# sneppy/pokerl

Measured on AMD Instinct MI355X. Metric: env-steps/sec (whole node) + showdown hand-evals/sec, 65 536 tables 6-max, higher is better.
Workload: dtype f64; 1 GPU; 65536 tables/GPU x 1 GPU(s), num_players=6, random agents in-kernel (Philox4x32-10), start_credits=100 blinds 1/2, auto-reset; BASELINE configs[2]; tables_per_gpu=65536, num_players=6, policy=random, kernel=k_rollout_tab<6> fused, 723 steps/launch, parallelism=env-parallel, 1 shard(s), no collective on the step path

## Files before the change

pokerl_amd/csrc/pk_device.hpp:

```cpp
#pragma once
#ifndef PK_HOST_SIM
#include <hip/hip_runtime.h>
#endif
#include <stdint.h>

#include <type_traits>
#include <utility>

#include "../../include/pokerl_hip.h"

namespace pk {

enum : int { HR_SF = 1, HR_POKER = 2, HR_FULL = 3, HR_FLUSH = 4, HR_STRAIGHT = 5, HR_TRIS = 6, HR_TWO_PAIR = 7, HR_PAIR = 8, HR_HIGH = 9, HR_NONE = 10 };
enum : int { MV_FOLD = 0, MV_CHECK = 1, MV_CALL = 2, MV_RAISE_ANY = 3, MV_ALL_IN = 6 };
enum : int { PS_FOLDED = 0, PS_ACTIVE = 1, PS_CALLED = 2, PS_ALL_IN = 3, PS_BROKEN = 4 };
constexpr uint32_t STREAM_DECK = 0x4445434Bu, STREAM_ACTION = 0x41435432u;
constexpr uint32_t NONE_V = (uint32_t)HR_NONE << 20;

constexpr int EVAL7_TAB_WORDS = 8192;

struct State {
    double *credits, *bets, *pending, *payoffs;
    double *min_raise;
    uint64_t *seat_states;
// ... 484 lines not shown
__device__ __forceinline__ uint32_t eval_tab_bits(uint64_t bits, const uint32_t *T, int &nk) {
    const Eval7Front f = eval7_tab_front_bits(bits, T);
    return eval_tab_back<SEVEN, true>(f, T, nk);
}
template <bool SEVEN = false>
__device__ __forceinline__ bool tab_bits_of(uint64_t w, int n, uint64_t &bits) {
    uint32_t lo = (uint32_t)w, hi = (uint32_t)(w >> 32) & 0x00ffffffu;
    if (!SEVEN) {
        const uint32_t r4 = rep4(lo), ulo = n >= 4 ? 0xffffffffu : ((1u << ((8 * n) & 31)) - 1u);
        const uint32_t uhi = n <= 4 ? 0u : ((1u << ((8 * (n - 4)) & 31)) - 1u);
        lo = (lo & ulo) | (r4 & ~ulo); hi = ((hi & uhi) | (r4 & ~uhi)) & 0x00ffffffu;
    }
    bits = (4ull << (lo & 63)) | (4ull << ((lo >> 8) & 63)) | (4ull << ((lo >> 16) & 63)) | (4ull << ((lo >> 24) & 63)) |
           (4ull << (hi & 63)) | (4ull << ((hi >> 8) & 63)) | (4ull << ((hi >> 16) & 63));
    const bool cards_ok = ((lo & 0xc0c0c0c0u) | (hi & 0x00c0c0c0u)) == 0 && (((uint32_t)bits | (uint32_t)(bits >> 32)) & 0x80038003u) == 0;
    return (SEVEN || n >= 3) && cards_ok && __popcll(bits) == (SEVEN ? 7 : n);
}
__device__ __forceinline__ uint32_t eval_small(uint64_t w, int n, int &nk) {
    uint32_t r0 = (uint32_t)w & 0xf, r1 = (uint32_t)(w >> 8) & 0xf;
    r0 = r0 ? r0 : 13u; r1 = r1 ? r1 : 13u;
    const uint32_t hi = r0 > r1 ? r0 : r1, lo = r0 > r1 ? r1 : r0;
    const bool pair = n == 2 && r0 == r1;
    nk = n == 0 ? 0 : ((n == 1 || pair) ? 1 : 2);
    const uint32_t v2 = pair ? (((uint32_t)HR_PAIR << 20) | r0) : (((uint32_t)HR_HIGH << 20) | (hi << 4) | lo);
    return n == 0 ? NONE_V : (n == 1 ? (((uint32_t)HR_HIGH << 20) | r0) : v2);
}
__device__ __forceinline__ uint32_t eval_tab_n(const uint32_t (&c)[7], int n, const uint32_t *T, int &nk) {
    uint64_t bits = 0;
#pragma unroll
    for (int i = 0; i < 7; ++i) bits |= (i < n) ? (4ull << (c[i] & 63)) : 0ull;
    return eval_tab_bits(bits, T, nk);
}
__device__ __forceinline__ bool distinct_valid_cards(const uint32_t (&c)[7], int n) {
    uint64_t bits = 0;
    bool ok = n >= 3;
#pragma unroll
    for (int i = 0; i < 7; ++i) {
        const bool used = i < n;
        ok = ok && (!used || (c[i] < 0x40u && (c[i] & 15u) < 13u));
        bits |= used ? (1ull << (c[i] & 63)) : 0ull;
    }
    return ok && __popcll(bits) == n;
}

#ifndef PK_WAVE
#define PK_WAVE 64
#endif
#define PK_STOCK (PK_WAVE >= 4 ? 4 : 1)
#if PK_WAVE >= 16
__device__ __forceinline__ uint32_t lane_read(uint32_t v, int lane) { return (uint32_t)__builtin_amdgcn_readlane((int)v, lane); }
__device__ __forceinline__ uint64_t lane_read64(uint64_t v, int lane) { return (uint64_t)lane_read((uint32_t)v, lane) | ((uint64_t)lane_read((uint32_t)(v >> 32), lane) << 32); }
__device__ __forceinline__ bool wave_uniform(bool b) { return __builtin_amdgcn_readfirstlane((int)b) != 0; }
#endif

enum : int { PF_ACTION = 0, PF_CURSOR = 1, PF_END_PRE = 2, PF_EVAL = 3, PF_SIDEPOT = 4, PF_SETUP = 5, PF_DEAL = 6, PF_OTHER = 7,
             PF_N_CURSOR = 8, PF_N_END = 9, PF_N_EVALPASS = 10, PF_N_SIDEPOT = 11,
             PF_N_SIDEPOT_LANES = 12, PF_N_END_LANES = 13, PF_SLOTS = 16 };
#ifdef PK_PROFILE
struct Prof {
    unsigned long long acc[PF_SLOTS] = {0}, t0 = 0;
    __device__ __forceinline__ void start() { t0 = __builtin_readcyclecounter(); }
    __device__ __forceinline__ void lap(int slot) { unsigned long long t = __builtin_readcyclecounter(); acc[slot] += t - t0; t0 = t; }
    __device__ __forceinline__ void count(int slot, unsigned n = 1) { acc[slot] += n; }
    __device__ __forceinline__ void count_wave(unsigned long long *dst, int slot_events, int slot_lanes) {
        const unsigned long long act = __ballot(1);
        if ((int)(threadIdx.x & 63) == __ffsll((long long)act) - 1) {
            atomicAdd(&dst[slot_events], 1ull); atomicAdd(&dst[slot_lanes], (unsigned long long)__popcll(act));
        }
    }
    __device__ __forceinline__ void flush(unsigned long long *dst) {
        if ((threadIdx.x & 63) == 0) for (int i = 0; i < PF_SLOTS; ++i) atomicAdd(&dst[i], acc[i]);
    }
};
#define PK_PROF(x) x
#else
#define PK_PROF(x)
#endif

template <int N>
struct Lds {
    static constexpr bool TAB = false;
    uint32_t item[64 * N + 64][2];
    uint32_t res[64 * N];
    uint32_t act[8][64];
    uint32_t show[N][64];
    Fresh fresh;
    alignas(16) uint8_t nth[128][8];
    uint32_t lone[(5 + 2 * N + 3) / 4];
    uint32_t stock[PK_STOCK][(5 + 2 * N + 3) / 4];
};

template <int N, bool RING>
struct LdsTab;
template <int N>
struct LdsTab<N, true> {
    static constexpr bool TAB = true, PAIRS = false;
    uint32_t item[64 * N + 1][2];
    uint32_t act[8][64];
    uint32_t show[N][64];
    Fresh fresh;
    alignas(16) uint8_t nth[128][8];
    alignas(16) uint32_t evtab[EVAL7_TAB_WORDS];
};
template <int N>
struct LdsTab<N, false> {
    static constexpr bool TAB = true, PAIRS = true;
// ... 26 lines not shown
    bool primed = false;
    template <typename LDS>
    __device__ __forceinline__ uint32_t draw16(LDS &lds, const Hot &S, uint32_t table_id, uint64_t step_serial, bool need) {
        const int lane = threadIdx.x & (PK_WAVE - 1);
        const uint64_t qfull = step_serial >> 3;
        const uint32_t q = (uint32_t)qfull;
        if (!primed || (int32_t)(filled - q) < 0) filled = q;
        primed = true;
        if (__any(need && filled == q)) {
#pragma unroll 1
            for (int r = 0; r < 2; ++r) {
                const bool fill = (int32_t)(filled - q) < 2;
                if (!__any(fill)) break;
                if (fill) {
                    const uint64_t b = qfull + (uint64_t)(filled - q);
                    uint32_t w[4];
                    philox4x32_10(table_id, (uint32_t)b, STREAM_ACTION, (uint32_t)(b >> 32), S.key0, S.key1, w);
                    const int slot = (filled & 1) * 4;
                    lds.act[slot + 0][lane] = w[0]; lds.act[slot + 1][lane] = w[1];
                    lds.act[slot + 2][lane] = w[2]; lds.act[slot + 3][lane] = w[3];
                    filled += 1;
                }
            }
        }
        const uint32_t j = (uint32_t)step_serial & 7;
        return lds.act[(q & 1) * 4 + (j >> 1)][lane];
    }
    template <typename LDS>
    __device__ __forceinline__ void ensure(LDS &lds, const Hot &S, uint32_t table_id, uint64_t step_serial, bool may, int ahead) {
        const int lane = threadIdx.x & (PK_WAVE - 1);
        const uint64_t qfull = step_serial >> 3;
        const uint32_t q = (uint32_t)qfull;
        if (!primed || (int32_t)(filled - q) < 0) filled = q;
        primed = true;
        const int have = (int)(filled - q) * 8 - (int)((uint32_t)step_serial & 7);
        if (__any(may && have < ahead)) {
#pragma unroll 1
            for (int r = 0; r < 2; ++r) {
                const bool fill = (int32_t)(filled - q) < 2;
                if (!__any(fill)) break;
                if (fill) {
                    const uint64_t b = qfull + (uint64_t)(filled - q);
                    uint32_t w[4];
                    philox4x32_10(table_id, (uint32_t)b, STREAM_ACTION, (uint32_t)(b >> 32), S.key0, S.key1, w);
                    const int slot = (filled & 1) * 4;
                    lds.act[slot + 0][lane] = w[0]; lds.act[slot + 1][lane] = w[1];
                    lds.act[slot + 2][lane] = w[2]; lds.act[slot + 3][lane] = w[3];
                    filled += 1;
                }
            }
        }
    }
    template <typename LDS>
    __device__ __forceinline__ static uint32_t peek(const LDS &lds, uint64_t step_serial) {
        const uint32_t s = (uint32_t)step_serial;
        return lds.act[((s >> 3) & 1) * 4 + ((s & 7) >> 1)][threadIdx.x & (PK_WAVE - 1)];
    }
    __device__ __forceinline__ static uint32_t half_of(uint32_t word, uint64_t step_serial) {
        return ((uint32_t)step_serial & 1) ? (word >> 16) : (word & 0xffffu);
    }
};
struct alignas(16) NthTable {
    uint8_t e[128][8];
    constexpr NthTable() : e{} {
        for (int m = 0; m < 128; ++m) {
            int rest = m;
            for (int k = 0; k < 8; ++k) {
                int low = 0;
                while (rest && !((rest >> low) & 1)) ++low;
                e[m][k] = rest ? (uint8_t)low : (uint8_t)0;
                rest &= rest - 1;
            }
        }
    }
};
__device__ __constant__ const NthTable g_nth{};
template <typename LDS>
__device__ __forceinline__ void stage_nth(LDS &lds) {
    static_assert(alignof(NthTable) >= 16 && sizeof(NthTable) == 64 * sizeof(uint4), "stage_nth copies the table as 64 uint4");
    for (int i = threadIdx.x & (PK_WAVE - 1); i < 64; i += PK_WAVE)
        reinterpret_cast<uint4 *>(&lds.nth[0][0])[i] = reinterpret_cast<const uint4 *>(&g_nth.e[0][0])[i];
    __syncthreads();
}
template <typename LDS>
__device__ __forceinline__ int action_from_draw_lds(const LDS &lds, uint32_t r16, uint32_t mask) {
    return lds.nth[mask & 127][__umul24(r16, (uint32_t)__popc(mask)) >> 16];
}
__device__ __forceinline__ int action_from_draw(uint32_t r16, uint32_t mask) {
    uint32_t k = __umul24(r16, (uint32_t)__popc(mask)) >> 16;
    uint32_t m = mask;
#pragma unroll
    for (uint32_t i = 0; i < 6; ++i) m = (i < k) ? (m & (m - 1)) : m;
    return __ffs(m) - 1;
}

__device__ __forceinline__ int call_action(uint32_t mask) {
    return ((mask >> MV_CALL) & 1) ? (int)MV_CALL : (((mask >> MV_CHECK) & 1) ? (int)MV_CHECK : (int)MV_ALL_IN);
}
__device__ __forceinline__ int pick_action(const Hot &S, ActionRng &rng, uint32_t table_id, uint64_t step_serial, uint32_t mask, int policy) {
    if (policy == PK_POLICY_ALLIN) return MV_ALL_IN;
    if (policy == PK_POLICY_CALL) return call_action(mask);
    return action_from_draw(rng.draw16(S, table_id, step_serial), mask);
}
__device__ __forceinline__ int seat_policy(uint64_t seatpol, int p) { return (int)((seatpol >> (4 * p)) & 15); }

#ifdef PK_HOST_SIM
#define PK_QSYNC() __syncthreads()
#else
#define PK_QSYNC() __builtin_amdgcn_wave_barrier()
#endif
template <int N>
struct Table {
// ... 166 lines not shown
        uint32_t over = 0;
        PK_FOR(p, N)
            over |= (pending[p] > credits[p]) ? (1u << p) : 0;
            pending[p] = (credits[p] < pending[p]) ? credits[p] : pending[p];
         PK_END
        st_active &= ~over; st_called &= ~over; st_broken &= ~over; st_allin |= over;
        min_raise = vmax<N>(pending);
        hands_this_step += 1;
    }
    __device__ __forceinline__ void reset_state(const Hot &S, int dealer_cfg) {
        dealer = dealer_cfg; hand = 0; active = 0;
        if (S.start_is_uniform) {
            PK_FOR(p, N) credits[p] = S.start_uniform; PK_END
        } else {
            PK_FOR(p, N) credits[p] = S.start_credits[p]; PK_END
        }
        st_active = FULL; st_called = st_allin = st_broken = 0;
        setup_state(S);
    }

    template <typename LDS>
    __device__ __forceinline__ void store_show(uint32_t *show, int T, int t, const LDS &lds) const {
        if (showed) {
            const int lane = threadIdx.x & (PK_WAVE - 1);
            const auto g_show = as_global(show);
            PK_FOR(p, N) g_show[(size_t)p * T + t] = lds.show[p][lane]; PK_END
        }
    }
    template <typename LDS>
    __device__ __forceinline__ static void stage_fresh(LDS &lds, const Fresh *src) {
        const int lane = threadIdx.x & (PK_WAVE - 1);
        constexpr int words = (int)(sizeof(Fresh) / 4);
        const auto s32 = as_global(reinterpret_cast<const uint32_t *>(src));
        uint32_t *d32 = reinterpret_cast<uint32_t *>(&lds.fresh);
        for (int i = lane; i < words; i += PK_WAVE) d32[i] = s32[i];
        __syncthreads();
    }
    template <typename LDS>
    __device__ __forceinline__ static void seed_dummy(LDS &lds) {
        if ((threadIdx.x & (PK_WAVE - 1)) == 0) {
            lds.item[64 * N][0] = 0x03020100u;
            lds.item[64 * N][1] = 4u | (5u << 6) | (6u << 12);
        }
    }
    __device__ __forceinline__ void load_fresh(const Fresh &f) {
        PK_FOR(p, N) credits[p] = f.credits[p]; bets[p] = 0.0; pending[p] = f.pending[p]; PK_END
        min_raise = f.min_raise;
        st_active = f.st_active; st_called = f.st_called; st_allin = f.st_allin; st_broken = f.st_broken;
        active = f.active; dealer = f.dealer; sb = f.sb; bb = f.bb;
        hand = 1; turn = 0;
        hands_this_step += 1;
    }

    __device__ __forceinline__ void begin_step(const Hot &S, int action, double high_bet) {
        const int a = active;
        const uint32_t b = 1u << a;
        hands_this_step = 0; terr = 0; flags = 0; stepped = 1;
        const bool money = action >= MV_CALL;
        const double credit = sel<N>(credits, a);
        const double base = (S.big_blind > high_bet) ? S.big_blind : high_bet;
        const double f = action == 3 ? 0.1 : (action == 4 ? 0.25 : 0.5);
        const double raised = base + (credit - base) * f;
        const bool is_raise = action >= MV_RAISE_ANY && action < MV_ALL_IN;
        const double bet_value = (action == MV_ALL_IN) ? credit : (is_raise ? raised : base);
        const bool raises = money && bet_value > high_bet;
        st_active |= raises ? st_called : 0;
        st_called = raises ? 0 : st_called;
        min_raise = raises ? bet_value - high_bet : min_raise;
        st_active &= ~b; st_called &= ~b; st_allin &= ~b; st_broken &= ~b;
        st_allin |= (action == MV_ALL_IN) ? b : 0;
        st_called |= (action != MV_FOLD && action != MV_ALL_IN) ? b : 0;
        PK_FOR(p, N) pending[p] = (money && p == a) ? bet_value : pending[p]; PK_END
        const bool many = __popc((st_active | st_called | st_allin) & FULL) > 1;
        current = a;
        active = many ? ((a + 1 == N) ? 0 : a + 1) : a;
        lstate = many ? LS_SCAN : LS_END;
        foldout = !many;
    }

    __device__ __forceinline__ bool scan() {
        int d = current - active; d = d < 0 ? d + N : d;
        uint32_t window = rotr(st_active, active) & ((2u << d) - 1);
        int a = active + (__ffs(window) - 1); a = a >= N ? a - N : a;
        active = window ? a : current;
        return window != 0;
    }
    __device__ __forceinline__ void cursor() {
        if (lstate != LS_SCAN) return;
        if (scan()) { lstate = LS_DONE; return; }
        next_turns();
    }
    __device__ __forceinline__ void scan_first() {
        int d = current - active; d = d < 0 ? d + N : d;
        uint32_t window = rotr(st_active, active) & ((2u << d) - 1);
        int a = active + (__ffs(window) - 1); a = a >= N ? a - N : a;
        const bool hit = lstate == LS_SCAN && window != 0;
        active = hit ? a : active;
        lstate = hit ? (int)LS_DONE : lstate;
    }
    __device__ __forceinline__ void cursor_tail() {
        if (lstate != LS_SCAN) return;
        active = current;
        next_turns();
    }
    __device__ __forceinline__ void next_turns() {
        PK_FOR(p, N) bets[p] = bets[p] + pending[p]; credits[p] = credits[p] - pending[p]; pending[p] = 0.0; PK_END
        min_raise = 0.0;
        turn += 1;
        const bool more = turn < 4;
        const bool merge = more && __popc(st_called) > 1;
        st_active |= merge ? st_called : 0u; st_called = merge ? 0u : st_called;
        const int first = first_playing(dealer + 1);
        int d = current - first; d = d < 0 ? d + N : d;
        const uint32_t window = rotr(st_active, first) & ((2u << d) - 1);
        int a = first + (__ffs(window) - 1); a = a >= N ? a - N : a;
        const bool found = more && window != 0;
        active = more ? (window ? a : current) : active;
        flags = more ? (uint32_t)PK_FLAG_TURN_OVER : flags;
        lstate = found ? LS_DONE : LS_END;
        turn = found ? turn : 4;
        foldout = false;
    }

    __device__ __forceinline__ bool parked() const { return lstate == LS_END || lstate == LS_POT; }

// ... 15 lines not shown
            PK_FOR(p, N)
                bets[p] = bets[p] + pending[p]; credits[p] = credits[p] - pending[p];
                pending[p] = 0.0; payoffs[p] = 0.0;
             PK_END
            min_raise = 0.0;
            uint32_t pw = (st_active | st_called | st_allin) & FULL;
            const int npw = __popc(pw);
            nowin = npw <= 0;
            {
                const int winner = (npw == 1) ? __ffs(pw) - 1 : -1;
                const double pot = np_sum<N>(bets);
                PK_FOR(p, N)
                    payoffs[p] = (p == winner) ? pot : payoffs[p];
                    credits[p] = (p == winner) ? credits[p] + pot : credits[p];
                 PK_END
            }
            sd = npw > 1;
            showdown = sd ? (st_called | st_allin) & FULL : 0u;
            pot_npw = sd ? npw : pot_npw;
        }
        PK_PROF(prof.lap(PF_END_PRE);)
        const int lane = threadIdx.x & 63;
        [[maybe_unused]] constexpr unsigned QN = sizeof(lds.item) / sizeof(lds.item[0]);
        bool lone = false;
#if PK_WAVE >= 16
        if constexpr (LONE) {
            const unsigned long long eb = __ballot(e);
            lone = __popcll(eb) == 1;
            if (lone) {
                const int sl = __ffsll((long long)eb) - 1;
                const uint32_t sm = lane_read(showdown, sl);
                if (sm) {
                    if (e) { PK_FOR(w, W) lds.lone[w] = cards[w]; PK_END }
                    __syncthreads();
                    const int q = lane < N ? lane : 0;
                    const uint8_t *lb = reinterpret_cast<const uint8_t *>(lds.lone);
                    const uint32_t c0 = lds.lone[0];
                    const uint32_t h[7] = {c0 & 0xff, (c0 >> 8) & 0xff, (c0 >> 16) & 0xff, c0 >> 24, lb[4],
                                           lb[5 + 2 * q], lb[6 + 2 * q]};
                    PK_QSYNC();
                    const uint32_t v = eval7_distinct(h);
                    uint32_t res[N];
                    PK_FOR(p, N) res[p] = lane_read(v, p); PK_END
                    if (sd) { PK_FOR(p, N) pot_hv[p] = ((showdown >> p) & 1) ? res[p] : NONE_V; PK_END }
                    evals += __popc(showdown);
                } else if (sd) {
                    PK_FOR(p, N) pot_hv[p] = NONE_V; PK_END
                }
            }
        }
#endif
        uint32_t total = 0, my_base[N];
        if (!lone) {
        PK_FOR(p, N)
            unsigned long long bal = __ballot((showdown >> p) & 1);
            my_base[p] = total + __builtin_amdgcn_mbcnt_hi((uint32_t)(bal >> 32), __builtin_amdgcn_mbcnt_lo((uint32_t)bal, 0u));
            total += (uint32_t)__popcll(bal);
         PK_END
        }
        if (lone) {
        } else if (total) {
            PK_FOR(p, N)
                const uint32_t slot = ((showdown >> p) & 1) ? my_base[p] : (uint32_t)(64 * N + (TAB ? 0 : lane));
                PK_DUMMY_STORE(TAB && !((showdown >> p) & 1), lds.item[PK_IDX(slot, QN, "lds.item")][0], cards[0]);
                PK_DUMMY_STORE(TAB && !((showdown >> p) & 1), lds.item[PK_IDX(slot, QN, "lds.item")][1], card(4) | (card(5 + 2 * p) << 6) | (card(6 + 2 * p) << 12) | (TAB ? 0u : ((uint32_t)(lane * N + p) << 18)));
             PK_END
            PK_QSYNC();
            uint32_t base0 = 0;
            if constexpr (TAB) {
                if constexpr (LDS::PAIRS) {
                    auto bits_of = [](uint32_t w0, uint32_t w1) {
                        return (4ull << (w0 & 63)) | (4ull << ((w0 >> 8) & 63)) | (4ull << ((w0 >> 16) & 63)) | (4ull << ((w0 >> 24) & 63)) |
                               (4ull << (w1 & 63)) | (4ull << ((w1 >> 6) & 63)) | (4ull << ((w1 >> 12) & 63));
                    };
                    for (; base0 + PK_WAVE < total; base0 += 2 * PK_WAVE) {
                        PK_PROF(prof.count(PF_N_EVALPASS, 2);)
                        const uint32_t ia = base0 + lane, ib0 = ia + PK_WAVE;
                        const uint32_t ib = ib0 < total ? ib0 : (uint32_t)(64 * N);
                        const uint32_t a0 = lds.item[PK_IDX(ia, QN, "lds.item")][0], a1 = lds.item[ia][1], b0 = lds.item[PK_IDX(ib, QN, "lds.item")][0], b1 = lds.item[ib][1];
                        const Eval7Front fa = eval7_tab_front_bits(bits_of(a0, a1), lds.evtab), fb = eval7_tab_front_bits(bits_of(b0, b1), lds.evtab);
                        const uint32_t va = eval7_tab_back(fa, lds.evtab), vb = eval7_tab_back(fb, lds.evtab);
                        lds.item[ia][0] = va;
                        if (ib0 < total) lds.item[ib][0] = vb;
                    }
                }
            }
            for (uint32_t base = base0; base < total; base += PK_WAVE) {
                PK_PROF(prof.count(PF_N_EVALPASS);)
                uint32_t i = base + lane;
                if (i < total) {
                    uint32_t w0 = lds.item[PK_IDX(i, QN, "lds.item")][0], w1 = lds.item[i][1];
                    if constexpr (TAB) {
                        const uint64_t bits = (4ull << (w0 & 63)) | (4ull << ((w0 >> 8) & 63)) | (4ull << ((w0 >> 16) & 63)) | (4ull << ((w0 >> 24) & 63)) |
                                              (4ull << (w1 & 63)) | (4ull << ((w1 >> 6) & 63)) | (4ull << ((w1 >> 12) & 63));
                        lds.item[i][0] = eval7_tab_back(eval7_tab_front_bits(bits, lds.evtab), lds.evtab);
                    } else {
                        uint32_t h[7] = {w0 & 0xff, (w0 >> 8) & 0xff, (w0 >> 16) & 0xff, w0 >> 24, w1 & 0x3f, (w1 >> 6) & 0x3f, (w1 >> 12) & 0x3f};
                        lds.res[PK_IDX(w1 >> 18, 64u * N, "lds.res")] = eval7_distinct(h);
                    }
                }
            }
            PK_QSYNC();
            if constexpr (TAB) { if (sd) { PK_FOR(p, N) pot_hv[p] = ((showdown >> p) & 1) ? lds.item[PK_IDX(my_base[p], QN, "lds.item")][0] : NONE_V; PK_END } }
            else if (sd) { PK_FOR(p, N) pot_hv[p] = ((showdown >> p) & 1) ? lds.res[PK_IDX(lane * N + p, 64 * N, "lds.res")] : NONE_V; PK_END }
            PK_QSYNC();
            evals += __popc(showdown);
        } else if (sd) {
            PK_FOR(p, N) pot_hv[p] = NONE_V; PK_END
        }
        PK_PROF(prof.lap(PF_EVAL);)
        PK_FOR(p, N) pot_wb[p] = sd ? bets[p] : pot_wb[p]; PK_END
// ... 124 lines not shown
```

pokerl_amd/csrc/pk_table_kernels.hpp:

```cpp
#pragma once
#ifndef PK_HOST_SIM
#include <hip/hip_runtime.h>
#endif

#include "pk_device.hpp"

using namespace pk;

#define PK_TABLE_BLOCK 64
static_assert(PK_TABLE_BLOCK == PK_WAVE, "one wavefront per workgroup: what PK_QSYNC (pk_device.hpp) and every wave-level ballot of the step machine assume");

template <typename ST>
__device__ __forceinline__ void wave_add_counters(const ST &S, uint32_t steps, uint32_t hands, uint32_t evals, uint32_t games) {
#pragma unroll
    for (int off = 32; off > 0; off >>= 1) {
        steps += __shfl_down(steps, off, 64); hands += __shfl_down(hands, off, 64);
        evals += __shfl_down(evals, off, 64); games += __shfl_down(games, off, 64);
    }
    if ((threadIdx.x & 63) == 0) {
        const auto slot = as_global(S.counters) + (size_t)blockIdx.x * PK_NUM_COUNTERS;
        slot[PK_C_STEPS] += steps; slot[PK_C_HANDS] += hands; slot[PK_C_EVALS] += evals; slot[PK_C_GAMES] += games;
    }
}

// ... 62 lines not shown
    f.min_raise = tb.min_raise;
    f.st_active = tb.st_active; f.st_called = tb.st_called; f.st_allin = tb.st_allin; f.st_broken = tb.st_broken;
    f.active = tb.active; f.dealer = tb.dealer; f.sb = tb.sb; f.bb = tb.bb;
    *out = f;
}

template <int N>
__global__ void __launch_bounds__(PK_TABLE_BLOCK) k_pick(State S, Hot H, int policy, int32_t *actions) {
    int t = blockIdx.x * H.tpb + threadIdx.x;
    if ((int)threadIdx.x >= H.tpb || t >= S.T) return;
    ActionRng rng;
    actions[t] = pick_action(H, rng, H.table_id_base + (uint32_t)t, S.step_serial[t], S.valid[t], policy);
}

struct StepKernArgs { const State *Sp; Hot H; const int32_t *actions; uint8_t *flags, *terr; int park, auto_reset; uint8_t *ready; int max_end;
                      double *obs; uint8_t *obs_packed; };
constexpr int PK_STEP_ROLLING = 16;
template <int N, bool ONE_PASS, int POLICY, int PASSES = 0, bool BOUNDED = false, bool TAB = false>
__device__ __forceinline__ void rollout_body(const State *__restrict__ Sp, const Hot &H, int K, int auto_reset, int park, int slack, int clear_terr,
                                             const int32_t *actions = nullptr, const StepKernArgs *ext = nullptr) {
    constexpr int policy = POLICY;
    const auto &S = *as_global(Sp);
    using LDS = std::conditional_t<TAB, LdsTab<N, POLICY == PK_POLICY_RANDOM>, Lds<N>>;
    PK_SHARED_OBJECT(LDS, lds);
    if constexpr (TAB) {
        static_assert(ONE_PASS && POLICY != PK_POLICY_EXTERNAL, "k_rollout_tab is a fused-rollout kernel");
#ifdef PK_HOST_SIM
        struct alignas(16) u32x4 { uint32_t v[4]; };
#else
        typedef uint32_t u32x4 __attribute__((ext_vector_type(4)));
#endif
        const auto g_tab = (PK_GLOBAL const u32x4 *)as_global(S.evtab);
        const int lane0 = threadIdx.x & (PK_WAVE - 1);
#pragma unroll 1
        for (int i = lane0; i < EVAL7_TAB_WORDS / 4; i += 8 * PK_WAVE) {
            u32x4 v[8];
#pragma unroll
            for (int j = 0; j < 8; ++j) v[j] = g_tab[i + j * PK_WAVE];
#pragma unroll
            for (int j = 0; j < 8; ++j) reinterpret_cast<u32x4 *>(lds.evtab)[i + j * PK_WAVE] = v[j];
        }
    }
    const int t = blockIdx.x * H.tpb + threadIdx.x;
    const bool live = (int)threadIdx.x < H.tpb && t < S.T;
    const uint32_t table_id = H.table_id_base + (uint32_t)t;
    Table<N> tb;
    uint32_t owed = 0;
    if constexpr (TAB) { if constexpr (LDS::PAIRS) Table<N>::seed_dummy(lds); }
    Table<N>::stage_fresh(lds, H.fresh);
    if constexpr (!TAB || POLICY == PK_POLICY_RANDOM) stage_nth(lds);
    constexpr bool EXTERNAL = POLICY == PK_POLICY_EXTERNAL;
    constexpr bool PAY = PASSES != 1;
    if (live) { tb.template load<PAY>(S, t); tb.hands_this_step = (int)as_global(S.mid)[t]; owed = as_global(S.owed)[t] + (uint32_t)K; } else tb.blank();
    uint32_t steps = 0;
    bool alive = live;
    ActionRing ring;
    double high_bet;
    int ext_action = -1;
    bool ext_ok = true;
    static_assert(!BOUNDED || POLICY == PK_POLICY_EXTERNAL, "bounded launches are pk_step_async_d's");
    if (EXTERNAL) {
        const uint32_t vm = tb.valid_mask(high_bet);
        if constexpr (BOUNDED) ext_action = (live && actions) ? as_global(actions)[t] : -1;
        else ext_action = live ? as_global(actions)[t] : -1;
        const bool carried = BOUNDED && live && tb.stepped;
        ext_ok = carried || (live && ext_action >= 0 && ext_action < PK_NUM_MOVES && ((vm >> ext_action) & 1));
        owed = ext_ok ? 1u : 0u;
        alive = ext_ok;
    }
    int nend = 0;
    uint32_t late = (live ? 1u : 0u) | (ext_ok ? 2u : 0u);
    if (EXTERNAL) PK_PIN_VGPR(late);
    const int cap = __popcll(__ballot(live && (owed > 0 || tb.lstate == LS_END)));
    const int quit = max(1, cap - slack);
    PK_PROF(tb.prof.start();)
    auto retire = [&]() {
        const bool r = tb.stepped && tb.lstate == LS_DONE;
        const bool bad = r && tb.terr != 0;
        const bool good = r && tb.terr == 0;
        tb.step_serial += (r && !(tb.terr & PK_TERR_NO_WINNER)) ? 1u : 0u;
        tb.stepped = r ? 0u : tb.stepped;
        owed = bad ? 0u : owed - (r ? 1u : 0u);
        alive = alive && !bad;
        steps += good ? 1u : 0u;
        tb.games += good ? (tb.flags & PK_FLAG_GAME_OVER) : 0u;
    };
    constexpr int PK_TAIL_MASK = 0xA;
    constexpr int PK_BET_PASSES = 4;
    static_assert((PK_TAIL_MASK >> (PK_BET_PASSES - 1)) & 1, "the last betting pass must run cursor_tail()");
    constexpr int NPASS = PASSES > 0 ? PASSES : PK_BET_PASSES;
    constexpr int TAILS = PASSES > 0 ? (1 << (PASSES - 1)) | (PK_TAIL_MASK & ((1 << PASSES) - 1)) : PK_TAIL_MASK;
    for (;;) {
        if (policy == PK_POLICY_RANDOM) __builtin_amdgcn_s_waitcnt(0);
        if constexpr (policy == PK_POLICY_RANDOM) ring.ensure(lds, H, table_id, tb.step_serial, alive && owed > 0, NPASS);
#pragma unroll
        for (int pass = 0; pass < NPASS; ++pass) {
            const bool go = alive && tb.lstate == LS_DONE && owed > 0;
            uint32_t word = 0;
            if constexpr (policy == PK_POLICY_RANDOM) word = ActionRing::peek(lds, tb.step_serial);
            if (go) {
                uint32_t mask = tb.valid_mask(high_bet);
                int act;
                if constexpr (EXTERNAL) act = ext_action;
                else if constexpr (policy == PK_POLICY_ALLIN) act = (int)MV_ALL_IN;
                else if constexpr (policy == PK_POLICY_CALL) act = call_action(mask);
                else act = action_from_draw_lds(lds, ActionRing::half_of(word, tb.step_serial), mask);
                tb.begin_step(H, act, high_bet);
            }
            PK_PROF(tb.prof.lap(PF_ACTION);)
            tb.scan_first();
            if ((TAILS >> pass) & 1) tb.cursor_tail();
            PK_PROF(tb.prof.count(PF_N_CURSOR);)
            retire();
            PK_PROF(tb.prof.lap(PF_CURSOR);)
        }
        const int parked = __popcll(__ballot(tb.parked()));
        const int runnable = __popcll(__ballot(alive && tb.lstate == LS_DONE && owed > 0));
        if (parked + runnable < quit) break;
        if (parked >= park || runnable == 0) {
            if constexpr (BOUNDED) {
                if (ext->max_end > 0 && nend >= ext->max_end && !__any(tb.stepped && tb.hands_this_step >= PK_STEP_ROLLING)) break;
                ++nend;
            }
            tb.template end_block<ONE_PASS>(H, t, table_id, lds, auto_reset != 0);
            retire();
        }
    }
    if (tb.lstate == LS_POT) { tb.lstate = LS_END; tb.evals -= (uint32_t)__popc((tb.st_called | tb.st_allin) & Table<N>::FULL); }
    if (EXTERNAL) {
        PK_PIN_VGPR(late);
        const bool ext_ok_l = late & 2u;
        if (late & 1u) {
            const auto flags_out = as_global(ext->flags), terr_out = as_global(ext->terr);
            const bool returned = !BOUNDED || !ext_ok_l || tb.lstate == LS_DONE;
            if (ext_ok_l) {
                tb.template store<PAY>(S, t);
                tb.store_show(S.show, S.T, t, lds);
                as_global(S.mid)[t] = returned ? 0u : (uint32_t)tb.hands_this_step;
                if (returned) as_global(S.valid)[t] = (uint8_t)tb.valid_mask(high_bet);
            }
            if (returned) {
                const uint8_t te = ext_ok_l ? (uint8_t)(tb.terr | tb.seen) : (uint8_t)PK_TERR_INVALID_ACTION;
                flags_out[t] = ext_ok_l ? (uint8_t)tb.flags : (uint8_t)0;
                as_global(S.terr)[t] = te;
                if (terr_out) terr_out[t] = te;
            }
            if constexpr (BOUNDED) as_global(ext->ready)[t] = returned ? 1 : 0;
            if (returned) {
                const auto obs = as_global(ext->obs);
                const auto obs_packed = as_global(ext->obs_packed);
                if (obs || obs_packed) {
                    const uint32_t vmask = tb.valid_mask(high_bet);
                    if (obs) write_obs_row<N>(tb, vmask, obs + (size_t)t * PK_OBS_DIM(N));
                    if (obs_packed) write_obs_packed_row<N>(tb, vmask, (PK_GLOBAL uint64_t *)(obs_packed + (size_t)t * PK_OBS_PACKED_BYTES(N)));
                }
            }
        }
        PK_PROF(tb.prof.flush(S.prof);)
        return;
    }
    if (live) {
        tb.template store<PAY>(S, t);
        tb.store_show(S.show, S.T, t, lds);
        as_global(S.owed)[t] = owed; as_global(S.mid)[t] = (uint32_t)tb.hands_this_step;
        as_global(S.valid)[t] = (uint8_t)tb.valid_mask(high_bet);
        const auto g_terr = as_global(S.terr);
        g_terr[t] = (uint8_t)((clear_terr ? 0 : g_terr[t]) | tb.terr | tb.seen);
    }
    wave_add_counters(S, steps, tb.hands, tb.evals, tb.games);
    PK_PROF(tb.prof.flush(S.prof);)
}

#define PK_WAVES_PER_SIMD_N(N) ((N) <= 12 ? 2 : 1)
template <int N>
__global__ void __launch_bounds__(PK_TABLE_BLOCK, PK_WAVES_PER_SIMD_N(N)) k_rollout(const State *__restrict__ Sp, Hot H, int K, int auto_reset, int park, int slack, int clear_terr) {
    rollout_body<N, true, PK_POLICY_RANDOM>(Sp, H, K, auto_reset, park, slack, clear_terr);
}
template <int N>
__global__ void __launch_bounds__(PK_TABLE_BLOCK, PK_WAVES_PER_SIMD_N(N)) k_rollout_tab(const State *__restrict__ Sp, Hot H, int K, int auto_reset, int park, int slack, int clear_terr) {
    rollout_body<N, true, PK_POLICY_RANDOM, 0, false, true>(Sp, H, K, auto_reset, park, slack, clear_terr);
}
template <int N>
__global__ void __launch_bounds__(PK_TABLE_BLOCK, PK_WAVES_PER_SIMD_N(N)) k_rollout_allin_tab(const State *__restrict__ Sp, Hot H, int K, int auto_reset, int park, int slack, int clear_terr) {
    rollout_body<N, true, PK_POLICY_ALLIN, 0, false, true>(Sp, H, K, auto_reset, park, slack, clear_terr);
}
template <int N>
__global__ void __launch_bounds__(PK_TABLE_BLOCK, PK_WAVES_PER_SIMD_N(N)) k_rollout_allin(const State *__restrict__ Sp, Hot H, int K, int auto_reset, int park, int slack, int clear_terr) {
    rollout_body<N, true, PK_POLICY_ALLIN>(Sp, H, K, auto_reset, park, slack, clear_terr);
}
template <int N>
__global__ void __launch_bounds__(PK_TABLE_BLOCK, PK_WAVES_PER_SIMD_N(N)) k_step(StepKernArgs) {
    const StepKernArgs *ka = (const StepKernArgs *)__builtin_amdgcn_kernarg_segment_ptr();
    const Hot H = ka->H;
    rollout_body<N, false, PK_POLICY_EXTERNAL, 1>(ka->Sp, H, 0, ka->auto_reset, ka->park, PK_WAVE, 1, ka->actions, ka);
}
template <int N>
__global__ void __launch_bounds__(PK_TABLE_BLOCK, PK_WAVES_PER_SIMD_N(N)) k_step_async(StepKernArgs) {
    const StepKernArgs *ka = (const StepKernArgs *)__builtin_amdgcn_kernarg_segment_ptr();
    Hot H = ka->H;
    asm volatile("" : "+s"(H.big_blind), "+s"(H.small_blind));
    rollout_body<N, false, PK_POLICY_EXTERNAL, 1, true>(ka->Sp, H, 0, ka->auto_reset, ka->park, PK_WAVE, 1, ka->actions, ka);
}
template <int N>
__global__ void __launch_bounds__(PK_TABLE_BLOCK, PK_WAVES_PER_SIMD_N(N)) k_rollout_single(const State *__restrict__ Sp, Hot H, int K, int auto_reset, int park, int slack, int clear_terr) {
    rollout_body<N, false, PK_POLICY_RANDOM, 1>(Sp, H, K, auto_reset, park, slack, clear_terr);
}
template <int N>
__global__ void __launch_bounds__(PK_TABLE_BLOCK, PK_WAVES_PER_SIMD_N(N)) k_rollout_call(const State *__restrict__ Sp, Hot H, int K, int auto_reset, int park, int slack, int clear_terr) {
    rollout_body<N, true, PK_POLICY_CALL>(Sp, H, K, auto_reset, park, slack, clear_terr);
}
constexpr int PK_OCC_CAP = 3;
template <int N>
__global__ void __launch_bounds__(PK_TABLE_BLOCK, PK_OCC_CAP) k_rollout_occ3(const State *__restrict__ Sp, Hot H, int K, int auto_reset, int park, int slack, int clear_terr) {
    rollout_body<N, true, PK_POLICY_RANDOM>(Sp, H, K, auto_reset, park, slack, clear_terr);
}
template <int N>
__global__ void __launch_bounds__(PK_TABLE_BLOCK, PK_OCC_CAP) k_rollout_occ3_allin(const State *__restrict__ Sp, Hot H, int K, int auto_reset, int park, int slack, int clear_terr) {
    rollout_body<N, true, PK_POLICY_ALLIN>(Sp, H, K, auto_reset, park, slack, clear_terr);
}


struct EnvResetKernArgs { const State *Sp; Hot H; const uint8_t *mask; uint64_t seatpol; int park; };
// ... 140 lines not shown
        phase = (int)(ctx >> 1) & 7; done = (ctx >> 4) & 1; hand = (ctx >> 5) & 1; terr_step = (uint32_t)(ctx >> 8) & 0xff;
        budget = (int)((ctx >> 16) & 0xffff) - 1; budget_reset = (int)((ctx >> 32) & 0xffff) - 1;
        rew = as_global(S.env_rew)[t];
        tb.hands_this_step = (int)as_global(S.mid)[t];
    }
    bool have_ext = MULTI && yielded && action_ok;
    const bool ext_invalid = MULTI && yielded && !action_ok;
    uint32_t late = (live ? 1u : 0u) | (ok ? 2u : 0u) | (carried ? 4u : 0u) | (skip ? 8u : 0u) | (ext_invalid ? 16u : 0u);
    asm volatile("" : "+v"(late));
    yielded = yielded && !have_ext;
    int passes = 0;
    const uint32_t caps = PK_TERR_HAND_CAP | PK_TERR_ENV_CAP;
    auto retire = [&]() {
        const bool r = tb.stepped && tb.lstate == LS_DONE;
        if (!__any(r)) return;
        tb.step_serial += (r && !(tb.terr & PK_TERR_NO_WINNER)) ? 1u : 0u;
        tb.stepped = r ? 0u : tb.stepped;
        const bool rp = r && phase == PH_RESET_PLAY;
        const bool opp = r && (phase == PH_HAND || phase == PH_TURN);
        budget_reset -= rp ? 1 : 0; budget -= opp ? 1 : 0;
        tb.terr |= ((rp && budget_reset < 0) || (opp && budget < 0)) ? (uint32_t)PK_TERR_ENV_CAP : 0u;
        const uint32_t idx = (uint32_t)phase | ((tb.flags & 3u) << 3) | (tb.terr != 0 ? 32u : 0u) | (tb.active == 0 ? 64u : 0u) | ((tb.st_broken & 1u) << 7);
        static_assert(PK_FLAG_GAME_OVER == 1 && PK_FLAG_HAND_OVER == 2, "env_transition()'s index takes the two flags as they are");
        const uint32_t w = r ? (uint32_t)trans[idx] : (uint32_t)phase;
        done = (w & 8u) ? (w >> 4) & 1u : done;
        hand = (w & 32u) ? (w >> 6) & 1u : hand;
        rew = (w & 128u) ? tb.payoffs[0] : rew;
        const bool fin = (w & 256u) != 0;
        terr_step = fin ? tb.terr : terr_step;
        phase = fin ? ((auto_reset && (done || (tb.terr & caps))) ? (int)PH_RESET : (int)PH_END) : (int)(w & 7u);
    };
    constexpr int PK_ENV_PASSES = 4;
    constexpr int PK_ENV_ROLLING = 16;
    constexpr int PK_ENV_PASSES_SYNC = 8;
    constexpr int EP = ASYNC ? PK_ENV_PASSES : PK_ENV_PASSES_SYNC;
    bool draws = seat0_policy == PK_POLICY_RANDOM;
    PK_FOR(p, N) if (p > 0) draws = draws || seat_policy(seatpol, p) == PK_POLICY_RANDOM; PK_END
    for (;;) {
        const bool closing = ASYNC && max_passes > 0 && passes >= max_passes;
        const bool last = closing && !__any(tb.stepped && tb.hands_this_step >= PK_ENV_ROLLING);
        PK_PROF(tb.prof.lap(PF_CURSOR);)
        if (!closing && phase == PH_RESET && tb.lstate == LS_DONE) {
            tb.reset_state(ka->H, 0); tb.deal(H, table_id);
            phase = tb.active != 0 ? PH_RESET_PLAY : PH_END;
        }
        PK_PROF(tb.prof.lap(14);)
        if (draws) __builtin_amdgcn_s_waitcnt(0);
        if (draws && !closing) ring.ensure(lds, H, table_id, tb.step_serial, phase != PH_END && !yielded, EP);
        PK_PROF(tb.prof.lap(15);)
        int made = 0;
#pragma unroll
        for (int pass = 0; pass < EP; ++pass) {
            const bool open = !(ASYNC && max_passes > 0 && passes + pass >= max_passes);
            const uint32_t word = draws ? ActionRing::peek(lds, tb.step_serial) : 0u;
            if (open && phase != PH_END && phase != PH_RESET && tb.lstate == LS_DONE && !yielded) {
                const uint32_t vm = tb.valid_mask(high_bet);
                const int pol = phase == PH_SEAT0 ? seat0_policy : seat_policy(seatpol, tb.active);
                const bool supplied = (phase == PH_SEAT0 && pol < 0) || (MULTI && phase != PH_SEAT0 && pol == PK_POLICY_EXTERNAL);
                const bool begin = !supplied || phase == PH_SEAT0 || have_ext;
                const int a_rand = draws ? action_from_draw_lds(lds, ActionRing::half_of(word, tb.step_serial), vm) : 0;
                const int a_call = call_action(vm);
                int a = pol == PK_POLICY_ALLIN ? (int)MV_ALL_IN : (pol == PK_POLICY_CALL ? a_call : a_rand);
                a = supplied ? action : a;
                if (MULTI && supplied && phase != PH_SEAT0) { yielded = !have_ext; have_ext = false; }
                if (begin) tb.begin_step(H, a, high_bet);
            }
            tb.cursor();
            retire();
            ++made;
            if (pass + 1 < EP &&
                !__any(phase != PH_END && phase != PH_RESET && tb.lstate == LS_DONE && !yielded)) break;
            if (ASYNC && max_passes > 0 && passes + pass + 1 >= max_passes) break;
        }
        PK_PROF(tb.prof.lap(PF_ACTION); tb.prof.count(PF_N_CURSOR, (unsigned)made);)
        const int parked = __popcll(__ballot(tb.parked()));
        const int runnable = closing ? 0 : __popcll(__ballot(phase != PH_END && tb.lstate == LS_DONE && !yielded));
        if (last || (parked == 0 && runnable == 0)) break;
        passes += made;
        if (parked >= park || runnable == 0) {
            tb.template end_block<false, !ASYNC>(H, t, table_id, lds, false);
            retire();
        }
    }
    PK_PROF(tb.prof.lap(PF_OTHER); tb.prof.flush(S.prof);)
    asm volatile("" : "+v"(late));
    const bool live_l = late & 1u, ok_l = late & 2u, carried_l = late & 4u, skip_l = late & 8u, ext_invalid_l = late & 16u;
    if (!live_l) return;
    const auto ready = as_global(ASYNC ? A.ready : nullptr), who_out = as_global(MULTI ? A.who : nullptr);
    const auto terr = as_global(A.terr);
    if (MULTI && skip_l) {
        if (ready) ready[t] = 3;
        if (who_out) who_out[t] = (uint8_t)tb.active;
        return;
    }
    if (ok_l) {
        tb.store(S, t);
        tb.store_show(S.show, S.T, t, lds);
    }
    const uint32_t vmask = tb.valid_mask(high_bet);
    const bool returned = !ASYNC || phase == PH_END;
    if (ASYNC) {
        const bool keep = !returned && !(MULTI && A.abandon);
        as_global(S.env_ctx)[t] = keep ? (1ull | ((uint64_t)phase << 1) | ((uint64_t)done << 4) | ((uint64_t)hand << 5) | ((uint64_t)(yielded ? 1 : 0) << 6) |
                                          ((uint64_t)(terr_step & 0xff) << 8) | ((uint64_t)(budget + 1) << 16) | ((uint64_t)(budget_reset + 1) << 32))
                                       : 0ull;
        as_global(S.mid)[t] = keep ? (uint32_t)tb.hands_this_step : 0u;
        as_global(S.valid)[t] = (uint8_t)vmask;
        if (ready) ready[t] = returned ? 1 : ((MULTI && yielded) ? 2 : 0);
        if (MULTI && who_out) who_out[t] = (uint8_t)tb.active;
        if (!returned) {
            as_global(S.env_rew)[t] = rew;
            if (!(MULTI && yielded) || !terr) return;
            terr[t] = ext_invalid_l ? (uint8_t)PK_TERR_INVALID_ACTION : (uint8_t)0;
// ... 45 lines not shown
```

Measured before the change: 29.65 billion env-steps/s.

## Trim per-lane bookkeeping in rollout loop and replace per-seat ballots with DPP scan

```diff
diff --git a/pokerl_amd/csrc/pk_device.hpp b/pokerl_amd/csrc/pk_device.hpp
--- a/pokerl_amd/csrc/pk_device.hpp
+++ b/pokerl_amd/csrc/pk_device.hpp
@@ -560,6 +560,23 @@
 __device__ __forceinline__ uint64_t lane_read64(uint64_t v, int lane) { return (uint64_t)lane_read((uint32_t)v, lane) | ((uint64_t)lane_read((uint32_t)(v >> 32), lane) << 32); }
 __device__ __forceinline__ bool wave_uniform(bool b) { return __builtin_amdgcn_readfirstlane((int)b) != 0; }
 #endif
+__device__ __forceinline__ uint32_t wave_excl_scan(uint32_t x, uint32_t &total) {
+#if PK_WAVE >= 16
+    static_assert(PK_WAVE == 64, "four rows of 16 lanes");
+    int s = (int)x;
+    s += __builtin_amdgcn_update_dpp(0, s, 0x111, 0xf, 0xf, true);
+    s += __builtin_amdgcn_update_dpp(0, s, 0x112, 0xf, 0xf, true);
+    s += __builtin_amdgcn_update_dpp(0, s, 0x114, 0xf, 0xf, true);
+    s += __builtin_amdgcn_update_dpp(0, s, 0x118, 0xf, 0xf, true);
+    s += __builtin_amdgcn_update_dpp(0, s, 0x142, 0xa, 0xf, false);
+    s += __builtin_amdgcn_update_dpp(0, s, 0x143, 0xc, 0xf, false);
+    total = lane_read((uint32_t)s, PK_WAVE - 1);
+    return (uint32_t)s - x;
+#else
+    total = x;
+    return 0u;
+#endif
+}
 
 enum : int { PF_ACTION = 0, PF_CURSOR = 1, PF_END_PRE = 2, PF_EVAL = 3, PF_SIDEPOT = 4, PF_SETUP = 5, PF_DEAL = 6, PF_OTHER = 7,
              PF_N_CURSOR = 8, PF_N_END = 9, PF_N_EVALPASS = 10, PF_N_SIDEPOT = 11,
@@ -692,12 +709,12 @@
         }
     }
     template <typename LDS>
-    __device__ __forceinline__ static uint32_t peek(const LDS &lds, uint64_t step_serial) {
-        const uint32_t s = (uint32_t)step_serial;
+    __device__ __forceinline__ static uint32_t peek(const LDS &lds, uint32_t step_serial) {
+        const uint32_t s = step_serial;
         return lds.act[((s >> 3) & 1) * 4 + ((s & 7) >> 1)][threadIdx.x & (PK_WAVE - 1)];
     }
-    __device__ __forceinline__ static uint32_t half_of(uint32_t word, uint64_t step_serial) {
-        return ((uint32_t)step_serial & 1) ? (word >> 16) : (word & 0xffffu);
+    __device__ __forceinline__ static uint32_t half_of(uint32_t word, uint32_t step_serial) {
+        return (step_serial & 1) ? (word >> 16) : (word & 0xffffu);
     }
 };
 struct alignas(16) NthTable {
@@ -970,6 +987,7 @@
         hands_this_step += 1;
     }
 
+    template <bool MONEY_IN_SEAT = false>
     __device__ __forceinline__ void begin_step(const Hot &S, int action, double high_bet) {
         const int a = active;
         const uint32_t b = 1u << a;
@@ -988,7 +1006,8 @@
         st_active &= ~b; st_called &= ~b; st_allin &= ~b; st_broken &= ~b;
         st_allin |= (action == MV_ALL_IN) ? b : 0;
         st_called |= (action != MV_FOLD && action != MV_ALL_IN) ? b : 0;
-        PK_FOR(p, N) pending[p] = (money && p == a) ? bet_value : pending[p]; PK_END
+        const int a_m = (!MONEY_IN_SEAT || money) ? a : -1;
+        PK_FOR(p, N) pending[p] = ((MONEY_IN_SEAT || money) && p == a_m) ? bet_value : pending[p]; PK_END
         const bool many = __popc((st_active | st_called | st_allin) & FULL) > 1;
         current = a;
         active = many ? ((a + 1 == N) ? 0 : a + 1) : a;
@@ -1110,11 +1129,8 @@
 #endif
         uint32_t total = 0, my_base[N];
         if (!lone) {
-        PK_FOR(p, N)
-            unsigned long long bal = __ballot((showdown >> p) & 1);
-            my_base[p] = total + __builtin_amdgcn_mbcnt_hi((uint32_t)(bal >> 32), __builtin_amdgcn_mbcnt_lo((uint32_t)bal, 0u));
-            total += (uint32_t)__popcll(bal);
-         PK_END
+            const uint32_t lane_base = wave_excl_scan((uint32_t)__popc(showdown), total);
+            PK_FOR(p, N) my_base[p] = lane_base + (uint32_t)__popc(showdown & ((1u << p) - 1u)); PK_END
         }
         if (lone) {
         } else if (total) {
diff --git a/pokerl_amd/csrc/pk_table_kernels.hpp b/pokerl_amd/csrc/pk_table_kernels.hpp
--- a/pokerl_amd/csrc/pk_table_kernels.hpp
+++ b/pokerl_amd/csrc/pk_table_kernels.hpp
@@ -138,8 +138,6 @@
     constexpr bool EXTERNAL = POLICY == PK_POLICY_EXTERNAL;
     constexpr bool PAY = PASSES != 1;
     if (live) { tb.template load<PAY>(S, t); tb.hands_this_step = (int)as_global(S.mid)[t]; owed = as_global(S.owed)[t] + (uint32_t)K; } else tb.blank();
-    uint32_t steps = 0;
-    bool alive = live;
     ActionRing ring;
     double high_bet;
     int ext_action = -1;
@@ -152,7 +150,6 @@
         const bool carried = BOUNDED && live && tb.stepped;
         ext_ok = carried || (live && ext_action >= 0 && ext_action < PK_NUM_MOVES && ((vm >> ext_action) & 1));
         owed = ext_ok ? 1u : 0u;
-        alive = ext_ok;
     }
     int nend = 0;
     uint32_t late = (live ? 1u : 0u) | (ext_ok ? 2u : 0u);
@@ -160,16 +157,16 @@
     const int cap = __popcll(__ballot(live && (owed > 0 || tb.lstate == LS_END)));
     const int quit = max(1, cap - slack);
     PK_PROF(tb.prof.start();)
+    uint32_t owed_base = owed;
+    static_assert(PK_TERR_NO_WINNER == 2 && PK_FLAG_GAME_OVER == 1, "retire()'s bit arithmetic");
     auto retire = [&]() {
-        const bool r = tb.stepped && tb.lstate == LS_DONE;
-        const bool bad = r && tb.terr != 0;
-        const bool good = r && tb.terr == 0;
-        tb.step_serial += (r && !(tb.terr & PK_TERR_NO_WINNER)) ? 1u : 0u;
-        tb.stepped = r ? 0u : tb.stepped;
-        owed = bad ? 0u : owed - (r ? 1u : 0u);
-        alive = alive && !bad;
-        steps += good ? 1u : 0u;
-        tb.games += good ? (tb.flags & PK_FLAG_GAME_OVER) : 0u;
+        const uint32_t r = tb.lstate == LS_DONE ? tb.stepped : 0u;
+        const uint32_t good = tb.terr == 0 ? r : 0u;
+        tb.step_serial += r & ~(tb.terr >> 1);
+        tb.stepped -= r;
+        owed -= r;
+        tb.games += good & tb.flags;
+        if (r != good) { owed_base -= owed + 1u; owed = 0u; }
     };
     constexpr int PK_TAIL_MASK = 0xA;
     constexpr int PK_BET_PASSES = 4;
@@ -178,20 +175,20 @@
     constexpr int TAILS = PASSES > 0 ? (1 << (PASSES - 1)) | (PK_TAIL_MASK & ((1 << PASSES) - 1)) : PK_TAIL_MASK;
     for (;;) {
         if (policy == PK_POLICY_RANDOM) __builtin_amdgcn_s_waitcnt(0);
-        if constexpr (policy == PK_POLICY_RANDOM) ring.ensure(lds, H, table_id, tb.step_serial, alive && owed > 0, NPASS);
+        if constexpr (policy == PK_POLICY_RANDOM) ring.ensure(lds, H, table_id, tb.step_serial, owed > 0, NPASS);
 #pragma unroll
         for (int pass = 0; pass < NPASS; ++pass) {
-            const bool go = alive && tb.lstate == LS_DONE && owed > 0;
+            const bool go = tb.lstate == LS_DONE && owed > 0;
             uint32_t word = 0;
-            if constexpr (policy == PK_POLICY_RANDOM) word = ActionRing::peek(lds, tb.step_serial);
+            if constexpr (policy == PK_POLICY_RANDOM) word = ActionRing::peek(lds, (uint32_t)tb.step_serial);
             if (go) {
                 uint32_t mask = tb.valid_mask(high_bet);
                 int act;
                 if constexpr (EXTERNAL) act = ext_action;
                 else if constexpr (policy == PK_POLICY_ALLIN) act = (int)MV_ALL_IN;
                 else if constexpr (policy == PK_POLICY_CALL) act = call_action(mask);
-                else act = action_from_draw_lds(lds, ActionRing::half_of(word, tb.step_serial), mask);
-                tb.begin_step(H, act, high_bet);
+                else act = action_from_draw_lds(lds, ActionRing::half_of(word, (uint32_t)tb.step_serial), mask);
+                tb.template begin_step<true>(H, act, high_bet);
             }
             PK_PROF(tb.prof.lap(PF_ACTION);)
             tb.scan_first();
@@ -201,7 +198,7 @@
             PK_PROF(tb.prof.lap(PF_CURSOR);)
         }
         const int parked = __popcll(__ballot(tb.parked()));
-        const int runnable = __popcll(__ballot(alive && tb.lstate == LS_DONE && owed > 0));
+        const int runnable = __popcll(__ballot(tb.lstate == LS_DONE && owed > 0));
         if (parked + runnable < quit) break;
         if (parked >= park || runnable == 0) {
             if constexpr (BOUNDED) {
@@ -253,7 +250,7 @@
         const auto g_terr = as_global(S.terr);
         g_terr[t] = (uint8_t)((clear_terr ? 0 : g_terr[t]) | tb.terr | tb.seen);
     }
-    wave_add_counters(S, steps, tb.hands, tb.evals, tb.games);
+    wave_add_counters(S, owed_base - owed, tb.hands, tb.evals, tb.games);
     PK_PROF(tb.prof.flush(S.prof);)
 }
 
@@ -500,13 +497,13 @@
 #pragma unroll
         for (int pass = 0; pass < EP; ++pass) {
             const bool open = !(ASYNC && max_passes > 0 && passes + pass >= max_passes);
-            const uint32_t word = draws ? ActionRing::peek(lds, tb.step_serial) : 0u;
+            const uint32_t word = draws ? ActionRing::peek(lds, (uint32_t)tb.step_serial) : 0u;
             if (open && phase != PH_END && phase != PH_RESET && tb.lstate == LS_DONE && !yielded) {
                 const uint32_t vm = tb.valid_mask(high_bet);
                 const int pol = phase == PH_SEAT0 ? seat0_policy : seat_policy(seatpol, tb.active);
                 const bool supplied = (phase == PH_SEAT0 && pol < 0) || (MULTI && phase != PH_SEAT0 && pol == PK_POLICY_EXTERNAL);
                 const bool begin = !supplied || phase == PH_SEAT0 || have_ext;
-                const int a_rand = draws ? action_from_draw_lds(lds, ActionRing::half_of(word, tb.step_serial), vm) : 0;
+                const int a_rand = draws ? action_from_draw_lds(lds, ActionRing::half_of(word, (uint32_t)tb.step_serial), vm) : 0;
                 const int a_call = call_action(vm);
                 int a = pol == PK_POLICY_ALLIN ? (int)MV_ALL_IN : (pol == PK_POLICY_CALL ? a_call : a_rand);
                 a = supplied ? action : a;
```

Result: faster. 30.54 billion env-steps/s (median of 6 runs) (+3.0%).
